# krukah/robopoker

Measured on AMD Instinct MI355X. Metric: mccfr_infoset_updates_per_sec, higher is better.
Workload: dtype f32; 1 GPU; leduc-holdem external-sampling MCCFR, tables resident in HBM (BASELINE configs[1]); regret=floored, weight=linear, sampling=external, batch_per_gpu=8388608, global_batch=8388608, infosets=120, actions=2, update=composed, parallelism=tree-sharded x1

## Files before the change

robopoker_amd/csrc/mccfr.hip:

```cpp
#include "mccfr_kernels.hpp"
#include "mccfr_traverse.hpp"
#include "mccfr_update.hpp"
#include "traverse_static.hpp"

#include <algorithm>
#include <chrono>
#include <cstdlib>
#include <functional>
#include <string>
#include <type_traits>
#include <vector>

#define HIP_TRY(expr)                                                                                 \
    do {                                                                                              \
        hipError_t _e = (expr);                                                                       \
        if (_e != hipSuccess) return rp::fail(RP_ERR_HIP, "%s failed: %s", #expr, hipGetErrorString(_e)); \
    } while (0)

using namespace rp;

struct KernelClock {
    std::vector<std::pair<hipEvent_t, hipEvent_t>> pending;
    double total_ms = 0.0;
    uint64_t launches = 0;
// ... 254 lines not shown
                std::vector<uint32_t>& rows, uint32_t* base, uint32_t* fan) {
    constexpr Skeleton S = SkelOf<G>::S;
    constexpr RowLayout R = SkelOf<G>::R;
    std::vector<std::vector<int>> kids(S.n);
    for (int s = 1; s < S.n; ++s) kids[S.parent[s]].push_back(s);
    for (int s = 0; s < S.n; ++s) fan[s] = base[s] = 0;
    bool uniform = true;
    std::function<void(uint32_t, int)> fans = [&](uint32_t sid, int s) {
        const rp_state& st = game->states[sid];
        if (S.kind[s] == SK_CHANCE) {
            if (fan[s] == 0) fan[s] = st.n_children;
            else if (fan[s] != st.n_children) uniform = false;
            for (uint32_t k = 0; k < st.n_children; ++k) fans(children[st.offset + k], kids[s][0]);
        } else if (S.kind[s] != SK_TERMINAL) {
            for (int c : kids[s]) fans(children[st.offset + (uint32_t)S.edge[c]], c);
        }
    };
    fans(game->train_root, 0);
    if (!uniform) return false;
    uint64_t total = 0;
    for (int c = 0; c < S.n; ++c) {
        if (S.kind[c] != SK_CHANCE) continue;
        uint64_t count = 1;
        for (int a = 0; a <= c; ++a)
            if (S.kind[a] == SK_CHANCE && c <= S.end[a]) count *= fan[a];
        base[c] = (uint32_t)(total / 4);
        total += (count * (uint64_t)R.stride[c] + 31) & ~(uint64_t)31;
        if (total > (1ull << 28)) return false;
    }
    rows.assign(total, 0u);
    std::function<void(uint32_t, int, uint64_t)> fill = [&](uint32_t sid, int s, uint64_t idx) {
        const rp_state& st = game->states[sid];
        if (const int c = R.group[s]; c >= 0) {
            uint32_t* row = &rows[(size_t)base[c] * 4 + idx * (uint64_t)R.stride[c]];
            const uint4 r = rec_of(sid);
            if (S.kind[s] == SK_CHANCE) {
                row[R.word[s]] = r.w;
                row[R.word2[s]] = r.y;
            } else if (S.kind[s] == SK_TERMINAL) {
                row[R.word[s]] = r.y;
                row[R.word2[s]] = r.z;
            } else {
                row[R.word[s]] = r.y;
            }
        }
        if (S.kind[s] == SK_CHANCE) {
            for (uint32_t k = 0; k < st.n_children; ++k) fill(children[st.offset + k], kids[s][0], idx * fan[s] + k);
        } else if (S.kind[s] != SK_TERMINAL) {
            for (int c : kids[s]) fill(children[st.offset + (uint32_t)S.edge[c]], c, idx);
        }
    };
    fill(game->train_root, 0, 0);
    return true;
}

size_t traverse_lds_bytes(const rp_mccfr* h) {
    const size_t shared = std::max<size_t>(2 * (size_t)h->maxint, 4 * (size_t)h->sc.maxs);
    return ((size_t)2 * h->sc.maxn + shared + (h->tbl.max_actions <= 4 ? 0 : h->tbl.max_actions)) * 64 * 4;
}
bool traverse_fits_lds(const rp_mccfr* h) {
    return h->sc.maxn <= 62 && h->maxint <= 32 && h->tbl.max_depth <= 10 && h->tbl.n_infos <= 8191 && h->tbl.max_actions <= 16 &&
           traverse_lds_bytes(h) <= 64 * 1024;
}

void launch_prepare_ref(rp_mccfr* h, const StepParams& p) {
    if (h->rng == RP_RNG_REFERENCE && h->ref_mid_epoch != p.epoch) {
        const uint32_t n = h->tbl.n_infos + h->n_chance_infos;
        rp_sip_mid* mid = reinterpret_cast<rp_sip_mid*>(h->d_ref_mid);
        hipLaunchKernelGGL(k_prepare_ref, dim3((n + 63) / 64), dim3(64), 0, h->stream, reinterpret_cast<const rp_hash_stream*>(h->d_info_streams),
                           h->tbl.n_infos, reinterpret_cast<const rp_hash_stream*>(h->d_chance_streams), h->n_chance_infos, p.epoch, mid,
                           mid + h->tbl.n_infos);
        h->ref_mid_epoch = p.epoch;
    }
}
void launch_prepare(rp_mccfr* h, const StepParams& p) {
    launch_prepare_ref(h, p);
    if (h->itab_version == h->tables_version) return;
    hipLaunchKernelGGL(k_prepare_infos, dim3((h->tbl.n_infos + 63) / 64), dim3(64), 0, h->stream, h->g, h->t, p, h->itab);
    h->itab_version = h->tables_version;
}

int launch_traverse(rp_mccfr* h, const StepParams& p) {
    if (h->dc.slotmap) HIP_TRY(hipMemsetAsync(h->dc.slotmap, 0, (size_t)h->tbl.n_infos * h->dc.stride, h->stream));
    clock_begin(h, h->clk_traverse);
    if (h->static_skel) {
        launch_prepare(h, p);
        const dim3 grid((h->batch + 255) / 256), block(256);
        with_static_traversal(h->static_skel, p.walker, p.S != RP_SAMPLING_EXTERNAL, p.ref_info != nullptr, [&](auto gt, auto wk, auto pr, auto rf) {
            hipLaunchKernelGGL((k_traverse_static<decltype(gt), decltype(wk)::value, decltype(pr)::value, decltype(rf)::value>), grid, block, 0,
                               h->stream, h->g, h->itab, h->dc, p);
        });
    } else if (h->use_lds_traverse) {
        launch_prepare(h, p);
        const size_t lds = traverse_lds_bytes(h);
        const dim3 grid((h->batch + 63) / 64), block(64);
        with_bool(h->tbl.max_actions <= 4, [&](auto tv) {
            hipLaunchKernelGGL((k_traverse_lds<decltype(tv)::value>), grid, block, lds, h->stream, h->g, h->itab, h->dc, p, h->sc.maxn, h->sc.maxs,
                               h->maxint);
        });
    } else {
        launch_prepare_ref(h, p);
        const uint32_t threads = 256, blocks = (h->batch + threads - 1) / threads;
        hipLaunchKernelGGL(k_traverse, dim3(blocks), dim3(threads), 0, h->stream, h->g, h->t, h->sc, h->dc, p);
    }
    clock_end(h, h->clk_traverse);
    HIP_TRY(hipGetLastError());
    return RP_OK;
}

int launch_sort(rp_mccfr* h, const StepParams& p) {
    const uint32_t nchunks = (h->batch + CH_TREES - 1) / CH_TREES;
    h->so.n_chunks = nchunks;
    clock_begin(h, h->clk_compact);
    if (!h->dc.slotmap) {
        const size_t NI = h->tbl.n_infos;
        hipLaunchKernelGGL(k_count_small, dim3(nchunks), dim3(CH_THREADS), NI * SM_WORDS * 4, h->stream, h->g, h->dc, h->so, p);
        hipLaunchKernelGGL(k_scan, dim3(h->tbl.n_infos), dim3(CH_THREADS), 0, h->stream, h->g, h->so, p);
        hipLaunchKernelGGL(k_compact_small, dim3(nchunks), dim3(CH_THREADS), NI * SM_WORDS * 4 + 2 * NI * 4 + NI * SM_WORDS * 2,
                           h->stream, h->g, h->dc, h->so, p);
    } else {
        hipLaunchKernelGGL(k_count, dim3(nchunks, h->tbl.n_infos), dim3(SLOT_THREADS), 0, h->stream, h->g, h->dc, h->so, p);
        hipLaunchKernelGGL(k_scan, dim3(h->tbl.n_infos), dim3(CH_THREADS), 0, h->stream, h->g, h->so, p);
        hipLaunchKernelGGL(k_compact, dim3(nchunks, h->tbl.n_infos), dim3(SLOT_THREADS), 0, h->stream, h->g, h->dc, h->so, p);
    }
    clock_end(h, h->clk_compact);
    HIP_TRY(hipGetLastError());
    return RP_OK;
}

int launch_chain(rp_mccfr* h, const StepParams& p) {
    const size_t lds = chain_lds_bytes();
    const bool sgn = h->R == RP_REGRET_DISCOUNTED || h->R == RP_REGRET_ASYMMETRIC;
    const bool prn = h->S != RP_SAMPLING_EXTERNAL;
    const dim3 grid(h->tbl.n_infos), block(128);
    clock_begin(h, h->clk_update);
    with_bools(sgn, prn, [&](auto sg, auto pr) {
        hipLaunchKernelGGL((k_chain<decltype(sg)::value, decltype(pr)::value>), grid, block, lds, h->stream, h->g, h->t, h->so, p);
    });
    clock_end(h, h->clk_update);
    HIP_TRY(hipGetLastError());
    return RP_OK;
}

uint32_t chunks_of(size_t trees) { return (uint32_t)((trees + RP_COMPOSE_CHUNK - 1) / RP_COMPOSE_CHUNK); }
size_t chunk_maps_lds_bytes(const rp_mccfr* h) {
    const size_t NI = h->tbl.n_infos;
    return NI * SM_WORDS * 4 + 2 * NI * 4 + (size_t)CH_TREES * h->maxdec * 4 + NI * SM_WORDS * 2 +
           2 * (size_t)CH_TREES * h->maxdec * 2;
}

size_t traverse_maps_lds_bytes(const rp_mccfr* h) {
    const size_t NI = h->tbl.n_infos;
    const size_t masks = h->S != RP_SAMPLING_EXTERNAL ? (size_t)h->maxdec * 256 * 4 : 0;
    return (NI * 8 + 2 * NI) * 4 + NI * 8 * 2 + (NI + (NI & 1)) * 2 + (size_t)5 * (h->maxdec * 256 + h->cell_pad) * 4 + masks;
}
static_assert(CH_THREADS <= 256u, "k_traverse_maps_static packs (infoset, rank of the infoset) into the 16 bits of an `order` entry");
bool traverse_maps_fused(const rp_mccfr* h) {
    return h->static_skel && !h->dc.slotmap && h->tbl.n_infos <= CH_THREADS && h->g.rank_max <= 64u &&
           traverse_maps_lds_bytes(h) <= 64 * 1024 && h->fuse_maps;
}

int launch_summarize(rp_mccfr* h, const StepParams& p, void* blob_dev, bool fused = false, bool apply = false) {
    unsigned char* blob = reinterpret_cast<unsigned char*>(blob_dev);
    Cell* cells = reinterpret_cast<Cell*>(blob);
    InfoSum* sums = reinterpret_cast<InfoSum*>(blob + (size_t)h->tbl.n_infos * h->tbl.max_actions * sizeof(Cell));
    const uint32_t A = h->tbl.max_actions;
    const uint32_t nblk_max = chunks_of(h->dc.stride), nblk = chunks_of(h->batch);
    Map* bmaps = reinterpret_cast<Map*>(h->d_bmaps);
    const bool pruned = h->S != RP_SAMPLING_EXTERNAL;
    if (fused) {
        clock_begin(h, h->clk_traverse);
        launch_prepare(h, p);
        const size_t lds = traverse_maps_lds_bytes(h);
        with_static_traversal(h->static_skel, p.walker, pruned, p.ref_info != nullptr, [&](auto gt, auto wk, auto pr, auto rf) {
            hipLaunchKernelGGL((k_traverse_maps_static<decltype(gt), decltype(wk)::value, decltype(pr)::value, decltype(rf)::value>), dim3(nblk),
                               dim3(256), lds, h->stream, h->g, h->itab, p, bmaps, h->maxdec, h->cell_pad);
        });
        clock_end(h, h->clk_traverse);
    }
    clock_begin(h, h->clk_update);
    if (fused) {
    } else if (!h->dc.slotmap) {
        const size_t lds = chunk_maps_lds_bytes(h);
        with_bools(pruned, h->tbl.n_infos <= CH_THREADS, [&](auto pr, auto one) {
            hipLaunchKernelGGL((k_chunk_maps<decltype(pr)::value, decltype(one)::value ? 1u : CM_PASSES>), dim3(nblk), dim3(CH_THREADS), lds,
                               h->stream, h->g, h->dc, p, bmaps);
        });
    } else {
        with_bool(pruned, [&](auto pr) {
            hipLaunchKernelGGL((k_block_maps<decltype(pr)::value>), dim3(nblk, h->tbl.n_infos), dim3(128), 0, h->stream, h->g, h->so, p, bmaps);
        });
    }
    {
        const uint32_t W2 = 2 * A, nr = h->g.rank_count[p.walker];
        const uint32_t ngrp_max = (nblk_max + RP_FOLD_GROUP - 1) / RP_FOLD_GROUP, ngrp = (nblk + RP_FOLD_GROUP - 1) / RP_FOLD_GROUP;
        FoldScratch fs;
        fs.gmaps = bmaps + bmap_index(nblk_max, 0, 0, h->g.rank_max, W2);
        fs.done = reinterpret_cast<uint32_t*>(bmaps + bmap_index(nblk_max + ngrp_max, 0, 0, h->g.rank_max, W2));
        const dim3 grid(std::max(ngrp, 1u), cb2_tiles(nr, W2));
        if (apply) {
            hipLaunchKernelGGL((k_combine2<true>), grid, dim3(CB2_THREADS), 0, h->stream, h->g, h->t, h->itab, p, bmaps, nr, fs, cells, sums);
            h->tables_version += 1;
            if (h->itab_version + 1 == h->tables_version) h->itab_version = h->tables_version;
        } else {
            hipLaunchKernelGGL((k_combine2<false>), grid, dim3(CB2_THREADS), 0, h->stream, h->g, h->t, h->itab, p, bmaps, nr, fs, cells, sums);
        }
    }
    clock_end(h, h->clk_update);
    HIP_TRY(hipGetLastError());
    return RP_OK;
}

int launch_batch_summary(rp_mccfr* h, const StepParams& p, void* blob_dev, bool apply = false) {
    if (traverse_maps_fused(h)) return launch_summarize(h, p, blob_dev, true, apply);
    int rc = launch_traverse(h, p);
    if (rc) return rc;
    if (h->dc.slotmap && (rc = launch_sort(h, p))) return rc;
    return launch_summarize(h, p, blob_dev, false, apply);
}

int enqueue_step(rp_mccfr* h) {
    const StepParams p = make_params(h);
    int rc;
    if (h->mode == RP_UPDATE_ORDERED) {
        if ((rc = launch_traverse(h, p))) return rc;
        if ((rc = launch_sort(h, p))) return rc;
        if ((rc = launch_chain(h, p))) return rc;
        h->tables_version += 1;
    } else {
        if ((rc = launch_batch_summary(h, p, h->d_summary, true))) return rc;
    }
    h->epoch += 1;
    return RP_OK;
}

int read_counters(rp_mccfr* h, unsigned long long c[3]) {
    std::vector<unsigned long long> all((size_t)METRIC_STRIPES * METRIC_STRIDE);
    HIP_TRY(hipMemcpyAsync(all.data(), h->d_counters, all.size() * 8, hipMemcpyDeviceToHost, h->stream));
    HIP_TRY(hipStreamSynchronize(h->stream));
    c[0] = c[1] = c[2] = 0;
    for (uint32_t s = 0; s < METRIC_STRIPES; ++s) {
        c[0] += all[(size_t)s * METRIC_STRIDE];
        c[1] += all[(size_t)s * METRIC_STRIDE + 1];
        c[2] |= all[(size_t)s * METRIC_STRIDE + 2];
    }
    return RP_OK;
}

int check_device_errors(rp_mccfr* h) {
    unsigned long long c[3];
    int rc = read_counters(h, c);
    if (rc) return rc;
    if (c[2]) return rp::fail(RP_ERR_CAPACITY, "mccfr kernel capacity exceeded (flags %llu): nodes/stack/decisions", c[2]);
    return RP_OK;
}

int composed_supported(const rp_mccfr* h) {
    if (h->R == RP_REGRET_DISCOUNTED || h->R == RP_REGRET_ASYMMETRIC)
        return rp::fail(RP_ERR_UNSUPPORTED,
                        "composed update needs a sign-independent discount (Summed/Linear/Floored regret)");
    return RP_OK;
}

int fetch_tables(rp_mccfr* h, std::vector<float>& regret, std::vector<float>& weight, std::vector<float>& payoff,
                 std::vector<uint32_t>& visits) {
    const size_t cells = (size_t)h->tbl.n_infos * h->tbl.max_actions;
    regret.resize(cells); weight.resize(cells); payoff.resize(cells); visits.resize(cells);
    HIP_TRY(hipMemcpyAsync(regret.data(), h->t.regret, cells * 4, hipMemcpyDeviceToHost, h->stream));
    HIP_TRY(hipMemcpyAsync(weight.data(), h->t.weight, cells * 4, hipMemcpyDeviceToHost, h->stream));
    HIP_TRY(hipMemcpyAsync(payoff.data(), h->t.payoff, cells * 4, hipMemcpyDeviceToHost, h->stream));
    HIP_TRY(hipMemcpyAsync(visits.data(), h->t.visits, cells * 4, hipMemcpyDeviceToHost, h->stream));
    HIP_TRY(hipStreamSynchronize(h->stream));
    return RP_OK;
}

}

extern "C" {

int rp_mccfr_create(const rp_game_table* game, rp_regret_kind r, rp_weight_kind w, rp_sampling_kind s,
                    uint32_t batch_size, const rp_hyper* hp, uint64_t seed, int device, rp_mccfr** out) {
    if (!game || !out) return rp::fail(RP_ERR_INVALID, "rp_mccfr_create: NULL argument");
    int rc = rp_game_table_check(game);
    if (rc) return rc;
    if ((int)r < 0 || (int)r > 4 || (int)w < 0 || (int)w > 3 || (int)s < 0 || (int)s > 2)
        return rp::fail(RP_ERR_INVALID, "rp_mccfr_create: unknown schedule / sampling kind");
    if (batch_size == 0) return rp::fail(RP_ERR_INVALID, "rp_mccfr_create: batch_size must be > 0");
    if (rp_device_count() <= 0)
        return rp::fail(RP_ERR_NO_DEVICE, "rp_mccfr_create: no HIP device visible; the MI355X path has no CPU fallback");
    if (game->max_tree_nodes == 0 || game->max_tree_nodes >= 255)
        return rp::fail(RP_ERR_CAPACITY, "rp_mccfr_create: sampled trees of up to %u nodes exceed the per-lane limit (254)",
                        game->max_tree_nodes);
    rp_mccfr* h = new rp_mccfr();
    h->device = device;
    h->tbl = *game;
    h->states.assign(game->states, game->states + game->n_states);
    h->children.assign(game->children, game->children + game->n_children);
    h->payoffs.assign(game->payoffs, game->payoffs + (size_t)game->n_terminals * game->n_players);
    h->info_actions.assign(game->info_actions, game->info_actions + game->n_infos);
    h->info_player.assign(game->info_player, game->info_player + game->n_infos);
    const size_t cells = (size_t)game->n_infos * game->max_actions;
    h->default_regret.assign(cells, 0.0f);
    if (game->default_regret) h->default_regret.assign(game->default_regret, game->default_regret + cells);
    h->tbl.states = h->states.data();
    h->tbl.children = h->children.data();
    h->tbl.payoffs = h->payoffs.data();
    h->tbl.info_actions = h->info_actions.data();
// ... 718 lines not shown
```

robopoker_amd/csrc/traverse_static.hpp:

```cpp
#pragma once

#include <type_traits>

#include "mccfr_kernels.hpp"
#include "mccfr_traverse.hpp"

namespace rp {

enum : int { SK_CHANCE = 0, SK_P0 = 1, SK_P1 = 2, SK_TERMINAL = 3 };
#define SK_MAXN 48

struct Skeleton {
    int n = 0;
    int kind[SK_MAXN] = {};
    int parent[SK_MAXN] = {};
    int edge[SK_MAXN] = {};
    int end[SK_MAXN] = {};
    constexpr int add(int k, int p, int e) {
        const int i = n++;
        kind[i] = k;
        parent[i] = p;
        edge[i] = e;
        end[i] = i;
        return i;
// ... 110 lines not shown
template <class G, int W, bool REF>
constexpr bool sk_slice_used(int c, int k) {
    constexpr Skeleton S = SkelOf<G>::S;
    constexpr RowLayout R = SkelOf<G>::R;
    for (int s = c + 1; s <= S.end[c]; ++s) {
        if (R.group[s] != c) continue;
        if (S.kind[s] == SK_TERMINAL) {
            if ((W == 0 ? R.word[s] : R.word2[s]) / 4 == k) return true;
        } else if (R.word[s] / 4 == k || (S.kind[s] == SK_CHANCE && REF && R.word2[s] / 4 == k)) {
            return true;
        }
    }
    return false;
}

template <class G>
constexpr bool sk_child_terminal(int s, int e) {
    for (int c = 0; c < SkelOf<G>::S.n; ++c)
        if (SkelOf<G>::S.parent[c] == s && SkelOf<G>::S.edge[c] == e) return SkelOf<G>::S.kind[c] == SK_TERMINAL;
    return false;
}

struct ExclPair {
    int lo = -1, hi = -1;
    int anc = -1;
    int edge_lo = 0;
};
constexpr int sk_lca(const Skeleton& S, int a, int b) {
    while (!(a <= b && b <= S.end[a])) a = S.parent[a];
    return a;
}
constexpr int sk_outer_edge(const Skeleton& S, int opp, int n, int k) {
    for (; S.parent[n] >= 0; n = S.parent[n])
        if (S.kind[S.parent[n]] == opp && k-- == 0) return S.parent[n] * 2 + S.edge[n];
    return -1;
}
constexpr bool sk_same_shape(const Skeleton& S, const RowLayout& R, int x, int y) {
    if (S.end[x] - x != S.end[y] - y || R.group[x] != R.group[y]) return false;
    for (int i = 0; i <= S.end[x] - x; ++i) {
        if (S.kind[x + i] != S.kind[y + i]) return false;
        if (i && (S.parent[x + i] - x != S.parent[y + i] - y || S.edge[x + i] != S.edge[y + i])) return false;
        if (i && (R.word[x + i] != R.word[y + i] || R.word2[x + i] != R.word2[y + i])) return false;
        if (S.kind[x + i] == SK_CHANCE && (R.words[x + i] != R.words[y + i] || R.stride[x + i] != R.stride[y + i])) return false;
    }
    return true;
}
constexpr ExclPair sk_exclusive_pair(const Skeleton& S, const RowLayout& R, int walker) {
    const int wk = walker == 0 ? SK_P0 : SK_P1, opp = walker == 0 ? SK_P1 : SK_P0;
    ExclPair best;
    bool best_even = false;
    for (int x = 0; x < S.n; ++x) {
        if (S.kind[x] != SK_CHANCE) continue;
        for (int y = S.end[x] + 1; y < S.n; ++y) {
            if (S.kind[y] != SK_CHANCE) continue;
            const int a = sk_lca(S, x, y);
            if (S.kind[a] != opp || !sk_same_shape(S, R, x, y)) continue;
            bool ordered = true;
            for (int n = S.end[x] + 1; n < y; ++n)
                if (S.kind[n] == wk && S.kind[sk_lca(S, x, n)] != opp) ordered = false;
            if (!ordered) continue;
            int kx = 0, ky = 0;
            while (sk_outer_edge(S, opp, x, kx) >= 0) ++kx;
            while (sk_outer_edge(S, opp, y, ky) >= 0) ++ky;
            if (best.lo >= 0 && (best_even || kx != ky)) continue;
            int c = x;
            while (S.parent[c] != a) c = S.parent[c];
            best.lo = x;
            best.hi = y;
            best.anc = a;
            best.edge_lo = S.edge[c];
            best_even = kx == ky;
        }
    }
    return best;
}
template <class G, int W, bool MERGE>
struct SkelExcl {
    using SK = SkelOf<G>;
    static constexpr ExclPair X = MERGE ? sk_exclusive_pair(SK::S, SK::R, W) : ExclPair{};
    static constexpr int LO = X.lo, HI = X.hi, SHIFT = X.hi - X.lo;
    static constexpr bool in_lo(int n) { return LO >= 0 && LO <= n && n <= SK::S.end[LO]; }
    static constexpr bool in_hi(int n) { return HI >= 0 && HI <= n && n <= SK::S.end[HI]; }
    static constexpr bool skipped(int n) { return in_lo(n) && n != LO; }
    static constexpr int at(int n) { return in_lo(n) ? n + SHIFT : n; }
    static constexpr bool both_below(int j) { return LO >= 0 && j < LO && HI <= SK::S.end[j]; }
};
template <class G>
constexpr bool sk_leaf_pair(int s) {
    int kids = 0;
    for (int c = 0; c < SkelOf<G>::S.n; ++c)
        if (SkelOf<G>::S.parent[c] == s) {
            if (SkelOf<G>::S.kind[c] != SK_TERMINAL) return false;
            ++kids;
        }
    return kids == 2;
}
template <class G>
constexpr int sk_child(int s, int e) {
    for (int c = 0; c < SkelOf<G>::S.n; ++c)
        if (SkelOf<G>::S.parent[c] == s && SkelOf<G>::S.edge[c] == e) return c;
    return -1;
}

static_assert(SkelOf<KuhnSkel>::S.n == 11, "Kuhn: two deals, four decision nodes, five terminals");
static_assert(SkelOf<LeducSkel>::S.n == 38, "Leduc: two deals, 4 + 3 x 4 decision nodes, three board draws, 2 + 3 x 5 terminals");
static_assert(SkelOf<LeducSkel>::S.end[0] == 37 && SkelOf<LeducSkel>::S.kind[2] == SK_P0, "pre-order, the first decision is P0's");
static_assert(SkelOf<LeducSkel>::R.words[0] == 2 && SkelOf<LeducSkel>::R.words[1] == 14 && SkelOf<LeducSkel>::R.stride[1] == 16,
              "Leduc: the second deal alone below the first; round 1 = 4 infosets, 3 board deals, 2 folds in a 64-byte row");
static_assert(SkelOf<KuhnSkel>::R.words[1] == 14 && SkelOf<KuhnSkel>::R.stride[1] == 16, "Kuhn: 4 infosets, 5 terminals");

static_assert(SkelExcl<LeducSkel, 0, true>::LO == 17 && SkelExcl<LeducSkel, 0, true>::HI == 28 && SkelExcl<LeducSkel, 0, true>::X.anc == 15 &&
                  SkelExcl<LeducSkel, 0, true>::X.edge_lo == 1,
              "Leduc, walker 0: CHECKED is the opponent's, so round 2 after check-raise-call and round 2 after check-check never meet");
static_assert(SkelExcl<LeducSkel, 1, true>::LO == 4 && SkelExcl<LeducSkel, 1, true>::HI == 28 && SkelExcl<LeducSkel, 1, true>::X.anc == 2 &&
                  SkelExcl<LeducSkel, 1, true>::X.edge_lo == 1,
              "Leduc, walker 1: OPEN is the opponent's; round 2 after raise-call pairs with the one after check-check (one opponent edge each)");
static_assert(SkelExcl<KuhnSkel, 0, true>::LO < 0 && SkelExcl<KuhnSkel, 1, true>::LO < 0, "Kuhn: one deal, nothing to pair");
static_assert(SkelExcl<LeducSkel, 0, false>::LO < 0 && !SkelExcl<LeducSkel, 0, false>::skipped(20) && SkelExcl<LeducSkel, 0, false>::at(20) == 20,
              "unmerged: every node stands for itself");
static_assert(sk_leaf_pair<LeducSkel>(6) && sk_leaf_pair<LeducSkel>(10) && !sk_leaf_pair<LeducSkel>(3) && sk_leaf_pair<KuhnSkel>(3) &&
                  sk_leaf_pair<KuhnSkel>(7),
              "fold / call below a raise: RAISED', CHECKRAISED' and Kuhn's Bet, CheckBet");

template <int I, int HI, class F>
__device__ __forceinline__ void sk_for(F&& f) {
    if constexpr (I < HI) {
        f(std::integral_constant<int, I>{});
        sk_for<I + 1, HI>(f);
    }
}
template <int I, int LO, class F>
__device__ __forceinline__ void sk_for_down(F&& f) {
    if constexpr (I >= LO) {
        f(std::integral_constant<int, I>{});
        sk_for_down<I - 1, LO>(f);
    }
}

template <class G, int W, bool PRUNED, bool REF, bool ROWS, class OnBuilt, class OnDecision>
__device__ __forceinline__ uint32_t static_traverse(const DevGame& g, const DevInfoTab& it, const StepParams& p, uint64_t tree_id,
                                                    bool present, OnBuilt&& on_built, OnDecision&& on_decision) {
    using SK = SkelOf<G>;
    using EX = SkelExcl<G, W, ROWS>;
    constexpr int N = SK::S.n;
    constexpr int K_WALKER = W == 0 ? SK_P0 : SK_P1;
    constexpr int K_OPP = W == 0 ? SK_P1 : SK_P0;

    uint32_t ry[N], rz[N], rw[N];
    uint32_t pay[N];
    uint32_t nout[N];
    uint32_t ridx[N];
    uint32_t pick[N];
    bool live[N];
    float sg0[N], sg1[N], q0[N], q1[N];
    bool sel_lo = false, live_lo = false, live_hi = false;
    const uint64_t th = rp_node_hash_tree(rp_node_hash_step(p.seed, p.epoch), tree_id);
    const char* const irows = reinterpret_cast<const char*>(it.row2);
    ry[0] = g.root_rec.y;
    rz[0] = g.root_rec.z;
    rw[0] = g.root_rec.w;
    live[0] = present;
    nout[0] = ROWS ? g.row_fan[0] : (g.root_rec.x >> 8) & 0xffu;
    sk_for<0, N>([&](auto I) __attribute__((always_inline)) {
        constexpr int s = I;
        constexpr int par = SK::S.parent[s];
        if constexpr (EX::skipped(s)) return;
        if constexpr (par >= 0) {
            if constexpr (!ROWS) {
                uint32_t k = (uint32_t)SK::S.edge[s];
                if constexpr (SK::S.kind[par] == SK_CHANCE) k = pick[par];
                const uint4 r = g.kids[rz[par] + k];
                ry[s] = r.y;
                rz[s] = r.z;
                rw[s] = r.w;
                pay[s] = W == 0 ? r.y : r.z;
                nout[s] = (r.x >> 8) & 0xffu;
            } else if constexpr (SK::S.kind[par] == SK_CHANCE) {
                constexpr int c = par;
                constexpr int up = SK::R.group[c];
                if constexpr (up >= 0) ridx[c] = ridx[up] * nout[c] + pick[c];
                else ridx[c] = pick[c];
                const char* row = reinterpret_cast<const char*>(g.rows + g.row_base[c]);
                uint32_t off = ridx[c] * (uint32_t)(SK::R.stride[c] * 4);
                if constexpr (EX::in_hi(c)) {
                    row = reinterpret_cast<const char*>(g.rows);
                    const uint32_t base_lo = g.row_base[c - EX::SHIFT], base_hi = g.row_base[c];
                    off += (sel_lo ? base_lo : base_hi) * 16u;
                }
                constexpr int NS = (SK::R.words[c] + 3) / 4;
                uint32_t w[NS * 4];
                sk_for<0, NS>([&](auto K) __attribute__((always_inline)) {
                    constexpr int k = K;
                    if constexpr (sk_slice_used<G, W, REF>(c, k)) {
                        const uint4 v = *reinterpret_cast<const uint4*>(row + off + (uint32_t)(k * 16));
                        w[4 * k + 0] = v.x;
                        w[4 * k + 1] = v.y;
                        w[4 * k + 2] = v.z;
                        w[4 * k + 3] = v.w;
                    }
                });
                sk_for<s, SK::S.end[c] + 1>([&](auto M) __attribute__((always_inline)) {
                    constexpr int m = M;
                    if constexpr (SK::R.group[m] == c) {
                        if constexpr (SK::S.kind[m] == SK_TERMINAL) {
                            pay[m] = w[W == 0 ? SK::R.word[m] : SK::R.word2[m]];
                        } else if constexpr (SK::S.kind[m] == SK_CHANCE) {
                            rw[m] = w[SK::R.word[m]];
                            if constexpr (REF) ry[m] = w[SK::R.word2[m]];
                            nout[m] = g.row_fan[m];
                            if constexpr (EX::in_hi(c)) {
                                const uint32_t fan_lo = g.row_fan[m - EX::SHIFT];
                                nout[m] = sel_lo ? fan_lo : nout[m];
                            }
                        } else {
                            ry[m] = w[SK::R.word[m]];
                        }
                    }
                });
            }
            if constexpr (SK::S.kind[par] == K_OPP) live[s] = live[par] && pick[par] == (uint32_t)SK::S.edge[s];
            else if constexpr (PRUNED && SK::S.kind[par] == K_WALKER) live[s] = live[par] && ((pick[par] >> SK::S.edge[s]) & 1u);
            else live[s] = live[par];
        }
        if constexpr (s == EX::LO) return;
        if constexpr (s == EX::HI) {
            sel_lo = pick[EX::X.anc] == (uint32_t)EX::X.edge_lo;
            live_lo = live[EX::LO];
            live_hi = live[s];
            const uint32_t key_lo = rw[EX::LO], key_hi = rw[s], fan_lo = nout[EX::LO], fan_hi = nout[s];
            rw[s] = sel_lo ? key_lo : key_hi;
            nout[s] = sel_lo ? fan_lo : fan_hi;
            if constexpr (REF) {
                const uint32_t ci_lo = ry[EX::LO], ci_hi = ry[s];
                ry[s] = sel_lo ? ci_lo : ci_hi;
            }
            live[s] = sel_lo ? live_lo : live_hi;
        }
        if constexpr (SK::S.kind[s] == SK_CHANCE) {
            if (REF && ry[s]) pick[s] = rp_ref_draw_range(rp_ref_seed_finish(&p.ref_chance[ry[s] - 1u], tree_id), nout[s]);
            else pick[s] = rp_pick_uniform(rp_node_hash_key(th, 0x80000000ull | rw[s]), nout[s]);
        } else if constexpr (SK::S.kind[s] == SK_P0 || SK::S.kind[s] == SK_P1) {
            const uint32_t info = ry[s];
            const char* const ir = irows + info * 32u;
            const float4 f = *reinterpret_cast<const float4*>(ir);
            sg0[s] = f.x;
            sg1[s] = f.y;
            q0[s] = f.z;
            q1[s] = f.w;
            if constexpr (SK::S.kind[s] == K_OPP) {
                const float2 tc = *reinterpret_cast<const float2*>(ir + 16);
                const float x = REF ? rp_ref_draw_weight(rp_ref_seed_finish(&p.ref_info[info], tree_id), tc.x)
                                    : rp_u01(rp_node_hash_key(th, info)) * tc.x;
                pick[s] = tc.y <= x ? 1u : 0u;
            } else if constexpr (PRUNED) {
                uint32_t mask = 3u;
                bool prune = true;
                if (p.S == RP_SAMPLING_PLURIBUS)
                    prune = p.epoch >= p.prune_warmup &&
                            !((REF ? rp_ref_draw_f32(rp_ref_seed_finish(&p.ref_info[info], tree_id)) : rp_u01(rp_node_hash_key(th, info))) <
                              p.prune_explore);
                if (prune) {
                    mask = *reinterpret_cast<const uint32_t*>(ir + 24) & 3u;
                    if (p.S == RP_SAMPLING_PLURIBUS)
                        mask |= (sk_child_terminal<G>(s, 0) ? 1u : 0u) | (sk_child_terminal<G>(s, 1) ? 2u : 0u);
                    mask = mask ? mask : 3u;
                }
                pick[s] = mask;
            }
        }
    });

    uint32_t nn = 0;
    sk_for<0, N>([&](auto I) __attribute__((always_inline)) {
        if constexpr (!EX::in_lo(decltype(I)::value)) nn += live[decltype(I)::value] ? 1u : 0u;
    });
    on_built([&](auto I) __attribute__((always_inline)) { return ry[EX::at(decltype(I)::value)]; },
             [&](auto I) __attribute__((always_inline)) { return EX::in_lo(decltype(I)::value) ? false : live[decltype(I)::value]; });
    sk_for<0, N>([&](auto J) __attribute__((always_inline)) {
        constexpr int j = J;
        if constexpr (SK::S.kind[j] == K_WALKER && !EX::in_lo(j)) {
            constexpr int E = SK::S.end[j];
            constexpr bool BOTH = EX::both_below(j);
            float rel[N], smp[N], acc[N], tv[2] = {0.0f, 0.0f};
            float rel_lo = 1.0f, smp_lo = 1.0f;
            sk_for<j + 1, E + 1>([&](auto Nn) __attribute__((always_inline)) {
                constexpr int n = Nn;
                constexpr int par = SK::S.parent[n];
                constexpr int e = SK::S.edge[n];
                constexpr int an = EX::at(n), ap = n == EX::LO ? par : EX::at(par);
                if constexpr (BOTH && EX::skipped(n)) return;
                float r = 1.0f, sm = 1.0f;
                if constexpr (ROWS && SK::S.kind[n] == SK_TERMINAL && SK::S.kind[par] == K_OPP && sk_leaf_pair<G>(par)) {
                    if constexpr (e == 1) {
                        const bool e1 = pick[ap] != 0u;
                        const float s_0 = sg0[ap], s_1 = sg1[ap], q_0 = q0[ap], q_1 = q1[ap];
                        constexpr int sib = EX::at(sk_child<G>(par, 0));
                        const uint32_t p_0 = pay[sib], p_1 = pay[an];
                        r = rel[ap] * (e1 ? s_1 : s_0);
                        sm = smp[ap] * (e1 ? q_1 : q_0);
                        const float v = r / sm * rp_u2f(e1 ? p_1 : p_0);
                        acc[ap] = live[ap] ? acc[ap] + v : acc[ap];
                    }
                    return;
                }
                if constexpr (par != j) {
                    r = rel[ap];
                    sm = smp[ap];
                    if constexpr (SK::S.kind[par] == K_WALKER) r = r * (e ? sg1[ap] : sg0[ap]);
                    if constexpr (SK::S.kind[par] == K_OPP) {
                        r = r * (e ? sg1[ap] : sg0[ap]);
                        sm = sm * (e ? q1[ap] : q0[ap]);
                    }
                }
                if constexpr (BOTH && n == EX::LO) {
                    rel_lo = r;
                    smp_lo = sm;
                    return;
                }
                if constexpr (BOTH && n == EX::HI) {
                    r = sel_lo ? rel_lo : r;
                    sm = sel_lo ? smp_lo : sm;
                }
                if constexpr (SK::S.kind[n] == SK_TERMINAL) {
                    const float v = r / sm * rp_u2f(pay[an]);
                    if constexpr (par == j) tv[e] = v;
                    else acc[ap] = live[an] ? acc[ap] + v : acc[ap];
                } else {
                    rel[an] = r;
                    smp[an] = sm;
                    acc[an] = 0.0f;
                }
            });
            sk_for_down<E, j + 1>([&](auto Nn) __attribute__((always_inline)) {
                constexpr int n = Nn;
                constexpr int par = SK::S.parent[n];
                constexpr int an = EX::at(n), ap = n == EX::LO ? par : EX::at(par);
                if constexpr (BOTH && EX::skipped(n)) return;
                if constexpr (SK::S.kind[n] != SK_TERMINAL) {
                    bool lv = live[an];
                    if constexpr (n == EX::LO) lv = live_lo;
                    if constexpr (n == EX::HI) lv = live_hi;
                    if constexpr (par == j) tv[SK::S.edge[n]] = acc[an];
                    else acc[ap] = lv ? acc[ap] + acc[an] : acc[ap];
                }
            });
            float cf = 1.0f, sm_ = 1.0f;
            sk_for<0, N>([&](auto Q) __attribute__((always_inline)) {
                constexpr int n = j - decltype(Q)::value;
                if constexpr (n > 0 && !(EX::in_hi(j) && n <= EX::HI)) {
                    if constexpr (n <= j && j <= SK::S.end[n]) {
                        constexpr int par = SK::S.parent[n];
                        if constexpr (SK::S.kind[par] == K_OPP) {
                            cf = cf * (SK::S.edge[n] ? sg1[par] : sg0[par]);
                            sm_ = sm_ * (SK::S.edge[n] ? q1[par] : q0[par]);
                        }
                    }
                }
            });
            if constexpr (EX::in_hi(j)) {
                sk_for<0, N>([&](auto Q) __attribute__((always_inline)) {
                    constexpr int fl = sk_outer_edge(SK::S, K_OPP, EX::LO, decltype(Q)::value);
                    constexpr int fh = sk_outer_edge(SK::S, K_OPP, EX::HI, decltype(Q)::value);
                    if constexpr (fl >= 0 || fh >= 0) {
                        float cl = 1.0f, ql = 1.0f, ch = 1.0f, qh = 1.0f;
                        if constexpr (fl >= 0) {
                            cl = (fl & 1) ? sg1[fl >> 1] : sg0[fl >> 1];
                            ql = (fl & 1) ? q1[fl >> 1] : q0[fl >> 1];
                        }
                        if constexpr (fh >= 0) {
                            ch = (fh & 1) ? sg1[fh >> 1] : sg0[fh >> 1];
                            qh = (fh & 1) ? q1[fh >> 1] : q0[fh >> 1];
                        }
                        cf = cf * (sel_lo ? cl : ch);
                        sm_ = sm_ * (sel_lo ? ql : qh);
                    }
                });
            }
            const float reach = cf / sm_;
            const float u0 = reach * tv[0], u1 = reach * tv[1];
            if constexpr (!PRUNED) {
                float ev = 0.0f;
                ev += sg0[j] * u0;
                ev += sg1[j] * u1;
                const float payoff = 0.0f + ev;
                const float g0 = 0.0f + (u0 - ev), g1 = 0.0f + (u1 - ev);
                if (live[j]) on_decision(J, ry[j], g0, g1, sg0[j], sg1[j], payoff, 3u);
            } else {
                const uint32_t mask = pick[j];
                float ev = 0.0f;
                if (mask & 1u) ev += sg0[j] * u0;
                if (mask & 2u) ev += sg1[j] * u1;
                const float payoff = 0.0f + ev;
                const float g0 = (mask & 1u) ? 0.0f + (u0 - ev) : 0.0f, g1 = (mask & 2u) ? 0.0f + (u1 - ev) : 0.0f;
                if (live[j]) on_decision(J, ry[j], g0, g1, sg0[j], sg1[j], payoff, mask);
            }
        }
    });
    return nn;
}

template <class G, int W, bool PRUNED, bool REF>
__global__ __launch_bounds__(256) void k_traverse_static(DevGame g, DevInfoTab it, DevDecisions dc, StepParams p) {
    const uint32_t lane = blockIdx.x * 256u + threadIdx.x;
    if (lane >= p.batch) return;
    const size_t D = dc.stride;
    uint32_t ndec = 0;
    auto on_built = [](auto, auto) __attribute__((always_inline)) {};
    auto on_decision =
        [&](auto, uint32_t info, float g0, float g1, float s0, float s1, float payoff, uint32_t mask) __attribute__((always_inline)) {
            const uint32_t slot = ndec;
            dc.regret[((size_t)slot * 2u + 0u) * D + lane] = g0;
            dc.regret[((size_t)slot * 2u + 1u) * D + lane] = g1;
            dc.policy[((size_t)slot * 2u + 0u) * D + lane] = s0;
            dc.policy[((size_t)slot * 2u + 1u) * D + lane] = s1;
            dc.info[(size_t)slot * D + lane] = info;
            dc.mask[(size_t)slot * D + lane] = mask;
            dc.payoff[(size_t)slot * D + lane] = payoff;
            if (dc.slotmap) dc.slotmap[(size_t)info * D + lane] = (uint8_t)(slot + 1u);
            ndec += 1u;
        };
    const uint64_t tree_id = p.tree_base + lane;
    const uint32_t nn = g.rows ? static_traverse<G, W, PRUNED, REF, true>(g, it, p, tree_id, true, on_built, on_decision)
                               : static_traverse<G, W, PRUNED, REF, false>(g, it, p, tree_id, true, on_built, on_decision);
    dc.ndec[lane] = (uint8_t)ndec;
    count_metrics(p, nn, ndec, 0u);
}

template <class G, int W, bool PRUNED, bool REF>
__global__ __launch_bounds__(256, 4) void k_traverse_maps_static(DevGame g, DevInfoTab it, StepParams p, Map* bmaps,
                                                              uint32_t maxdec, uint32_t lpad) {
    extern __shared__ __attribute__((aligned(16))) uint32_t tm_lds[];
    static_assert(SM_WORDS == 8u, "a bitmap row is two 16-byte LDS reads, its prefix counts two 8-byte writes");
    const uint32_t NI = g.n_infos, chunk = blockIdx.x, lt = threadIdx.x;
    const uint32_t nr = g.rank_count[W];
    const uint32_t my_info = lt < nr ? g.rank_info[(size_t)W * g.rank_max + lt] : 0u;
    uint32_t* bits = tm_lds;
    uint32_t* lcount = bits + NI * SM_WORDS;
    uint32_t* lbase = lcount + NI;
    uint16_t* pre = reinterpret_cast<uint16_t*>(lbase + NI);
    uint16_t* order = pre + NI * SM_WORDS;
    float* vals = reinterpret_cast<float*>(order + NI + (NI & 1u));
    const uint32_t L = maxdec * 256u + lpad;
    uint32_t* lmask = reinterpret_cast<uint32_t*>(vals + 5u * L);
    for (uint32_t e = lt; e < NI * SM_WORDS; e += 256u) bits[e] = 0;
    __syncthreads();
    const uint32_t lane = chunk * 256u + lt;
    const float tf = (float)p.epoch;
    uint32_t ndec = 0;
    auto on_built =
        [&](auto info_of, auto live_of) __attribute__((always_inline)) {
            sk_for<0, SkelOf<G>::S.n>([&](auto J) __attribute__((always_inline)) {
                if constexpr (SkelOf<G>::S.kind[decltype(J)::value] == (W == 0 ? SK_P0 : SK_P1)) {
                    if (live_of(J)) atomicOr(&bits[info_of(J) * SM_WORDS + (lt >> 5)], 1u << (lt & 31u));
                }
            });
            __syncthreads();
            if (lt < 64u) {
                const bool mine = lt < nr;
                uint2* const pw = reinterpret_cast<uint2*>(pre + my_info * SM_WORDS);
                const uint4 lo = *reinterpret_cast<const uint4*>(bits + my_info * SM_WORDS);
                const uint32_t p1 = __popc(lo.x), p2 = p1 + __popc(lo.y), p3 = p2 + __popc(lo.z), p4 = p3 + __popc(lo.w);
                if (mine) pw[0] = make_uint2(p1 << 16, p2 | p3 << 16);
                const uint4 hi = *reinterpret_cast<const uint4*>(bits + my_info * SM_WORDS + 4u);
                const uint32_t p5 = p4 + __popc(hi.x), p6 = p5 + __popc(hi.y), p7 = p6 + __popc(hi.z);
                if (mine) pw[1] = make_uint2(p4 | p5 << 16, p6 | p7 << 16);
                const uint32_t run = mine ? p7 + __popc(hi.w) : 0u;
                uint32_t incl = run;
                for (int d = 1; d < 64; d <<= 1) {
                    const uint32_t o = __shfl_up(incl, d, 64);
                    if ((int)lt >= d) incl += o;
                }
                const uint32_t len = run ? 32u - (uint32_t)__builtin_clz(run) : 0u;
                uint32_t place = 0, at = 0;
                for (uint32_t k = 10u; k-- > 0u;) {
                    const unsigned long long m = __ballot(mine && len == k);
                    if (len == k) place = at + __builtin_amdgcn_mbcnt_hi((uint32_t)(m >> 32), __builtin_amdgcn_mbcnt_lo((uint32_t)m, 0u));
                    at += (uint32_t)__popcll(m);
                }
                if (mine) {
                    lcount[my_info] = run;
                    lbase[my_info] = incl - run;
                    order[place] = (uint16_t)(my_info | lt << 8);
                }
            }
            __syncthreads();
        };
    auto on_decision =
        [&](auto, uint32_t info, float g0, float g1, float s0, float s1, float payoff, uint32_t mask) __attribute__((always_inline)) {
            const uint32_t pos = lbase[info] + list_rank(bits, pre, info, lt);
            if constexpr (PRUNED) lmask[pos] = mask;
            vals[pos] = g0;
            vals[L + pos] = g1;
            vals[2u * L + pos] = weight_delta(p.W, s0, tf);
            vals[3u * L + pos] = weight_delta(p.W, s1, tf);
            vals[4u * L + pos] = payoff;
            ndec += 1u;
        };
    const uint64_t tree_id = p.tree_base + lane;
    const bool present = lane < p.batch;
    const uint32_t nn = g.rows ? static_traverse<G, W, PRUNED, REF, true>(g, it, p, tree_id, present, on_built, on_decision)
                               : static_traverse<G, W, PRUNED, REF, false>(g, it, p, tree_id, present, on_built, on_decision);
    __syncthreads();
    const ChainParams cpr = chain_params(p, true, tf), cpw = chain_params(p, false, tf);
    if (cpr.d == 1.0f && cpw.d == 1.0f) {
        const uint32_t ln = lt & 63u, sub = ln / 5u, c = ln - 5u * sub;
        const float fl = c < 2u ? cpr.fl : (c < 4u ? cpw.fl : rp_u2f(0xff800000u));
        for (uint32_t i = (lt >> 6) * 12u + sub; ln < 60u && i < nr; i += 4u * 12u) {
            const uint32_t info = order[i] & 255u, rank = order[i] >> 8;
            const uint32_t n = lcount[info], base = lbase[info];
            const float* v = vals + (size_t)c * L + base;
            Map mp = map_identity();
            for (uint32_t e = 0; e < n; ++e) map_touch_unit_unless(mp, PRUNED && c < 2u && !((lmask[base + e] >> c) & 1u), v[e], fl);
            if (c == 4u) mp.b = 0.0f + mp.b;
            bmaps[bmap_index(chunk, rank, c, g.rank_max, 4u)] = mp;
        }
    } else {
        for (uint32_t task = lt; task < 5u * nr; task += 256u) {
            const uint32_t c = task < 4u * nr ? task & 3u : 4u;
            const uint32_t oi = order[task < 4u * nr ? task >> 2 : task - 4u * nr], info = oi & 255u, rank = oi >> 8;
            const uint32_t n = lcount[info], base = lbase[info];
            const size_t out = bmap_index(chunk, rank, c, g.rank_max, 4u);
            const float* v = vals + (size_t)c * L + base;
            if (c == 4u) {
                float sum = 0.0f;
                for (uint32_t e = 0; e < n; ++e) sum += v[e];
                bmaps[out] = map_sum_slot(sum, n);
                continue;
            }
            const bool isreg = c < 2u;
            const ChainParams cp = isreg ? cpr : cpw;
            Map mp = map_identity();
            for (uint32_t e = 0; e < n; ++e) map_touch_unless(mp, PRUNED && isreg && !((lmask[base + e] >> c) & 1u), cp.d, v[e], cp.fl);
            bmaps[out] = mp;
        }
    }
    count_metrics(p, nn, ndec, 0u);
}

}
```

Before: 74.62 billion infoset-updates/s.

## Store per-infoset strategy once and keep only chosen opponent probabilities

After: 81.69 billion infoset-updates/s (median of 6 runs). 1.09x the previous value.

```diff
diff --git a/robopoker_amd/csrc/mccfr.hip b/robopoker_amd/csrc/mccfr.hip
--- a/robopoker_amd/csrc/mccfr.hip
+++ b/robopoker_amd/csrc/mccfr.hip
@@ -430,7 +430,7 @@
 size_t traverse_maps_lds_bytes(const rp_mccfr* h) {
     const size_t NI = h->tbl.n_infos;
     const size_t masks = h->S != RP_SAMPLING_EXTERNAL ? (size_t)h->maxdec * 256 * 4 : 0;
-    return (NI * 8 + 2 * NI) * 4 + NI * 8 * 2 + (NI + (NI & 1)) * 2 + (size_t)5 * (h->maxdec * 256 + h->cell_pad) * 4 + masks;
+    return (NI * 8 + 2 * NI) * 4 + NI * 8 * 2 + (NI + (NI & 1)) * 2 + 2 * NI * 4 + (size_t)3 * (h->maxdec * 256 + h->cell_pad) * 4 + masks;
 }
 static_assert(CH_THREADS <= 256u, "k_traverse_maps_static packs (infoset, rank of the infoset) into the 16 bits of an `order` entry");
 bool traverse_maps_fused(const rp_mccfr* h) {
diff --git a/robopoker_amd/csrc/traverse_static.hpp b/robopoker_amd/csrc/traverse_static.hpp
--- a/robopoker_amd/csrc/traverse_static.hpp
+++ b/robopoker_amd/csrc/traverse_static.hpp
@@ -286,7 +286,8 @@
     uint32_t ridx[N];
     uint32_t pick[N];
     bool live[N];
-    float sg0[N], sg1[N], q0[N], q1[N];
+    float sg0[N], sg1[N];
+    float sgp[N], qp[N];
     bool sel_lo = false, live_lo = false, live_hi = false;
     const uint64_t th = rp_node_hash_tree(rp_node_hash_step(p.seed, p.epoch), tree_id);
     const char* const irows = reinterpret_cast<const char*>(it.row2);
@@ -376,17 +377,21 @@
         } else if constexpr (SK::S.kind[s] == SK_P0 || SK::S.kind[s] == SK_P1) {
             const uint32_t info = ry[s];
             const char* const ir = irows + info * 32u;
-            const float4 f = *reinterpret_cast<const float4*>(ir);
-            sg0[s] = f.x;
-            sg1[s] = f.y;
-            q0[s] = f.z;
-            q1[s] = f.w;
             if constexpr (SK::S.kind[s] == K_OPP) {
+                const float4 f = *reinterpret_cast<const float4*>(ir);
                 const float2 tc = *reinterpret_cast<const float2*>(ir + 16);
                 const float x = REF ? rp_ref_draw_weight(rp_ref_seed_finish(&p.ref_info[info], tree_id), tc.x)
                                     : rp_u01(rp_node_hash_key(th, info)) * tc.x;
-                pick[s] = tc.y <= x ? 1u : 0u;
-            } else if constexpr (PRUNED) {
+                const bool e1 = tc.y <= x;
+                pick[s] = e1 ? 1u : 0u;
+                sgp[s] = e1 ? f.y : f.x;
+                qp[s] = e1 ? f.w : f.z;
+            } else {
+                const float2 f = *reinterpret_cast<const float2*>(ir);
+                sg0[s] = f.x;
+                sg1[s] = f.y;
+            }
+            if constexpr (SK::S.kind[s] == K_WALKER && PRUNED) {
                 uint32_t mask = 3u;
                 bool prune = true;
                 if (p.S == RP_SAMPLING_PLURIBUS)
@@ -427,11 +432,10 @@
                 if constexpr (ROWS && SK::S.kind[n] == SK_TERMINAL && SK::S.kind[par] == K_OPP && sk_leaf_pair<G>(par)) {
                     if constexpr (e == 1) {
                         const bool e1 = pick[ap] != 0u;
-                        const float s_0 = sg0[ap], s_1 = sg1[ap], q_0 = q0[ap], q_1 = q1[ap];
                         constexpr int sib = EX::at(sk_child<G>(par, 0));
                         const uint32_t p_0 = pay[sib], p_1 = pay[an];
-                        r = rel[ap] * (e1 ? s_1 : s_0);
-                        sm = smp[ap] * (e1 ? q_1 : q_0);
+                        r = rel[ap] * sgp[ap];
+                        sm = smp[ap] * qp[ap];
                         const float v = r / sm * rp_u2f(e1 ? p_1 : p_0);
                         acc[ap] = live[ap] ? acc[ap] + v : acc[ap];
                     }
@@ -442,8 +446,8 @@
                     sm = smp[ap];
                     if constexpr (SK::S.kind[par] == K_WALKER) r = r * (e ? sg1[ap] : sg0[ap]);
                     if constexpr (SK::S.kind[par] == K_OPP) {
-                        r = r * (e ? sg1[ap] : sg0[ap]);
-                        sm = sm * (e ? q1[ap] : q0[ap]);
+                        r = r * sgp[ap];
+                        sm = sm * qp[ap];
                     }
                 }
                 if constexpr (BOTH && n == EX::LO) {
@@ -485,8 +489,8 @@
                     if constexpr (n <= j && j <= SK::S.end[n]) {
                         constexpr int par = SK::S.parent[n];
                         if constexpr (SK::S.kind[par] == K_OPP) {
-                            cf = cf * (SK::S.edge[n] ? sg1[par] : sg0[par]);
-                            sm_ = sm_ * (SK::S.edge[n] ? q1[par] : q0[par]);
+                            cf = cf * sgp[par];
+                            sm_ = sm_ * qp[par];
                         }
                     }
                 }
@@ -498,12 +502,12 @@
                     if constexpr (fl >= 0 || fh >= 0) {
                         float cl = 1.0f, ql = 1.0f, ch = 1.0f, qh = 1.0f;
                         if constexpr (fl >= 0) {
-                            cl = (fl & 1) ? sg1[fl >> 1] : sg0[fl >> 1];
-                            ql = (fl & 1) ? q1[fl >> 1] : q0[fl >> 1];
+                            cl = sgp[fl >> 1];
+                            ql = qp[fl >> 1];
                         }
                         if constexpr (fh >= 0) {
-                            ch = (fh & 1) ? sg1[fh >> 1] : sg0[fh >> 1];
-                            qh = (fh & 1) ? q1[fh >> 1] : q0[fh >> 1];
+                            ch = sgp[fh >> 1];
+                            qh = qp[fh >> 1];
                         }
                         cf = cf * (sel_lo ? cl : ch);
                         sm_ = sm_ * (sel_lo ? ql : qh);
@@ -560,8 +564,9 @@
     count_metrics(p, nn, ndec, 0u);
 }
 
+constexpr int tm_workgroups(bool pruned, bool ref) { return (!pruned && !ref) ? 5 : 4; }
 template <class G, int W, bool PRUNED, bool REF>
-__global__ __launch_bounds__(256, 4) void k_traverse_maps_static(DevGame g, DevInfoTab it, StepParams p, Map* bmaps,
+__global__ __launch_bounds__(256, tm_workgroups(PRUNED, REF)) void k_traverse_maps_static(DevGame g, DevInfoTab it, StepParams p, Map* bmaps,
                                                               uint32_t maxdec, uint32_t lpad) {
     extern __shared__ __attribute__((aligned(16))) uint32_t tm_lds[];
     static_assert(SM_WORDS == 8u, "a bitmap row is two 16-byte LDS reads, its prefix counts two 8-byte writes");
@@ -573,13 +578,13 @@
     uint32_t* lbase = lcount + NI;
     uint16_t* pre = reinterpret_cast<uint16_t*>(lbase + NI);
     uint16_t* order = pre + NI * SM_WORDS;
-    float* vals = reinterpret_cast<float*>(order + NI + (NI & 1u));
+    float* wsig = reinterpret_cast<float*>(order + NI + (NI & 1u));
+    float* vals = wsig + 2u * NI;
     const uint32_t L = maxdec * 256u + lpad;
-    uint32_t* lmask = reinterpret_cast<uint32_t*>(vals + 5u * L);
+    uint32_t* lmask = reinterpret_cast<uint32_t*>(vals + 3u * L);
     for (uint32_t e = lt; e < NI * SM_WORDS; e += 256u) bits[e] = 0;
     __syncthreads();
     const uint32_t lane = chunk * 256u + lt;
-    const float tf = (float)p.epoch;
     uint32_t ndec = 0;
     auto on_built =
         [&](auto info_of, auto live_of) __attribute__((always_inline)) {
@@ -621,13 +626,15 @@
         };
     auto on_decision =
         [&](auto, uint32_t info, float g0, float g1, float s0, float s1, float payoff, uint32_t mask) __attribute__((always_inline)) {
-            const uint32_t pos = lbase[info] + list_rank(bits, pre, info, lt);
+            const uint32_t at = list_rank(bits, pre, info, lt), pos = lbase[info] + at;
+            if (at == 0u) {
+                wsig[2u * info] = s0;
+                wsig[2u * info + 1u] = s1;
+            }
             if constexpr (PRUNED) lmask[pos] = mask;
             vals[pos] = g0;
             vals[L + pos] = g1;
-            vals[2u * L + pos] = weight_delta(p.W, s0, tf);
-            vals[3u * L + pos] = weight_delta(p.W, s1, tf);
-            vals[4u * L + pos] = payoff;
+            vals[2u * L + pos] = payoff;
             ndec += 1u;
         };
     const uint64_t tree_id = p.tree_base + lane;
@@ -635,16 +642,22 @@
     const uint32_t nn = g.rows ? static_traverse<G, W, PRUNED, REF, true>(g, it, p, tree_id, present, on_built, on_decision)
                                : static_traverse<G, W, PRUNED, REF, false>(g, it, p, tree_id, present, on_built, on_decision);
     __syncthreads();
+    const float tf = (float)p.epoch;
     const ChainParams cpr = chain_params(p, true, tf), cpw = chain_params(p, false, tf);
     if (cpr.d == 1.0f && cpw.d == 1.0f) {
         const uint32_t ln = lt & 63u, sub = ln / 5u, c = ln - 5u * sub;
         const float fl = c < 2u ? cpr.fl : (c < 4u ? cpw.fl : rp_u2f(0xff800000u));
+        const bool isw = c == 2u || c == 3u;
+        const uint32_t cell = c == 4u ? 2u : c & 1u;
         for (uint32_t i = (lt >> 6) * 12u + sub; ln < 60u && i < nr; i += 4u * 12u) {
             const uint32_t info = order[i] & 255u, rank = order[i] >> 8;
             const uint32_t n = lcount[info], base = lbase[info];
-            const float* v = vals + (size_t)c * L + base;
+            const float* v = vals + (size_t)cell * L + base;
+            const float wd = weight_delta(p.W, wsig[2u * info + (c & 1u)], tf);
+            const uint32_t keep = isw ? 0u : ~0u, own = isw ? rp_f2u(wd) : 0u;
             Map mp = map_identity();
-            for (uint32_t e = 0; e < n; ++e) map_touch_unit_unless(mp, PRUNED && c < 2u && !((lmask[base + e] >> c) & 1u), v[e], fl);
+            for (uint32_t e = 0; e < n; ++e)
+                map_touch_unit_unless(mp, PRUNED && c < 2u && !((lmask[base + e] >> c) & 1u), rp_u2f((rp_f2u(v[e]) & keep) | own), fl);
             if (c == 4u) mp.b = 0.0f + mp.b;
             bmaps[bmap_index(chunk, rank, c, g.rank_max, 4u)] = mp;
         }
@@ -654,8 +667,8 @@
             const uint32_t oi = order[task < 4u * nr ? task >> 2 : task - 4u * nr], info = oi & 255u, rank = oi >> 8;
             const uint32_t n = lcount[info], base = lbase[info];
             const size_t out = bmap_index(chunk, rank, c, g.rank_max, 4u);
-            const float* v = vals + (size_t)c * L + base;
             if (c == 4u) {
+                const float* v = vals + (size_t)2u * L + base;
                 float sum = 0.0f;
                 for (uint32_t e = 0; e < n; ++e) sum += v[e];
                 bmaps[out] = map_sum_slot(sum, n);
@@ -663,8 +676,12 @@
             }
             const bool isreg = c < 2u;
             const ChainParams cp = isreg ? cpr : cpw;
+            const float* v = vals + (size_t)(c & 1u) * L + base;
+            const float wd = weight_delta(p.W, wsig[2u * info + (c & 1u)], tf);
+            const uint32_t keep = isreg ? ~0u : 0u, own = isreg ? 0u : rp_f2u(wd);
             Map mp = map_identity();
-            for (uint32_t e = 0; e < n; ++e) map_touch_unless(mp, PRUNED && isreg && !((lmask[base + e] >> c) & 1u), cp.d, v[e], cp.fl);
+            for (uint32_t e = 0; e < n; ++e)
+                map_touch_unless(mp, PRUNED && isreg && !((lmask[base + e] >> c) & 1u), cp.d, rp_u2f((rp_f2u(v[e]) & keep) | own), cp.fl);
             bmaps[out] = mp;
         }
     }
```
